# david-cortes/recometrics

Measured on AMD Instinct MI355X. Metric: users/sec evaluated (all metrics, K=10), higher is better.
Workload: dtype f32

## Files before the change

### recometrics_amd/csrc/rm_finalize.hpp

```cpp
#pragma once
#include "rm_device.hpp"
#include <type_traits>

namespace rm {

constexpr int MAX_PARTS = 128;
constexpr int FIN_THREADS = 128;
constexpr int FIN_TOPV = 64;
template <class T> inline size_t finalize_lds_bytes(int K, int n_part) { return (sizeof(T) * (size_t)(K < FIN_TOPV ? K : FIN_TOPV) + 4 * (size_t)n_part) * FIN_THREADS; }

struct AucPart { unsigned long long sum_ranks; double s1, s2; int nvalid, pad; };

template <class T, class S> struct FinalArgs {
    int m, n, K, n_part, req, cumulative, noise, gu, n_slots;
    const int *slot_user, *slot_chunk;
    const int *train_p, *test_p, *test_i; const T *test_v;
    const int *flags, *user_nslots, *uslot_base, *slot_index;
    const int *gj; const long long *grow;
    const Entry<S> *pl; const PartialStat<S> *pst; const unsigned *hist; const S *pos_score;
    const int *pos_item_tab;
    AucPart *auc_part;
    T *heavy_topv;
    unsigned char *heavy_nan;
    const int *heavy_users; int n_heavy;
// ... 10 lines not shown
    int auc_defer_slot0;
    const S *stream_scores; long long stream_ld;
    const S *spos_score; const int *spos_item;
    unsigned *shist;
    int ext_topk; unsigned long long *sel_hi; unsigned *sel_lo; int sel_ld;
    int collected;
    int *noise_flag; Plan *plan;
};

template <class T> __device__ __forceinline__ T qnan();
template <> __device__ __forceinline__ float qnan<float>() { return __int_as_float(0x7fc00000); }
template <> __device__ __forceinline__ double qnan<double>() { return __longlong_as_double(0x7ff8000000000000ll); }

template <class T, class S>
__device__ void fill_user_nan(const FinalArgs<T, S> &a, int u)
{
    T *top8[8] = {a.p, a.tp, a.r, a.ap, a.tap, a.ndcg, a.hit, a.rr};
    for (int q = 0; q < 8; q++) {
        T *arr = top8[q];
        if (!arr) continue;
        if (!a.cumulative) arr[u] = qnan<T>();
        else for (int i = 0; i < a.K; i++) arr[(size_t)u * a.K + i] = qnan<T>();
    }
    if (a.roc) a.roc[u] = qnan<T>();
    if (a.pr) a.pr[u] = qnan<T>();
}

template <class S> __device__ __forceinline__ bool ent_before(const Entry<S> &x, const Entry<S> &y)
{
    return x.s > y.s || (x.s == y.s && x.idx < y.idx);
}

template <class T, class S>
__global__ void k_auc_slots(FinalArgs<T, S> a)
{
    const int slot = blockIdx.x * blockDim.x + threadIdx.x;
    if (slot >= a.stream_slot0) return;
    const int u = a.slot_user[slot], c = a.slot_chunk[slot];
    if (a.flags[u] & UF_ONLY_NDCG) return;
    const int te0 = a.test_p[u], npos = a.test_p[u + 1] - te0;
    const int GUr = a.gu;
    const int g = slot / GUr, ul = slot % GUr;
    const int PLg = (1 << a.gj[g]) - 1;
    const unsigned *H = a.hist + (a.grow[g] + g) * GUr + ul;
    const S *PS = a.pos_score + (a.grow[g] + g) * GUr + ul;
    const int pc = min(POS_CHUNK, npos - c * POS_CHUNK);
    unsigned long long above = 0, sum_ranks = 0;
    double s1 = 0, s2 = 0;
    int nvalid = 0;
    for (int b = PLg; b >= 1; b--) {
        above += H[(size_t)b * GUr];
        const int j = b - 1;
        if (j >= pc) continue;
        const S ps = PS[(size_t)j * GUr];
        if (isinf(ps) && ps > 0) continue;
        const unsigned long long rank = above + 1;
        sum_ranks += rank; nvalid++;
        s1 += 1. / (double)rank;
        s2 += (double)nvalid / (double)rank;
        if (a.rank_sorted) a.rank_sorted[te0 + c * POS_CHUNK + j] = (long long)rank;
    }
    AucPart r; r.sum_ranks = sum_ranks; r.s1 = s1; r.s2 = s2; r.nvalid = nvalid; r.pad = 0;
    a.auc_part[slot] = r;
}

constexpr int MERGE_WAVES = 4;
template <class T, class S>
__global__ __launch_bounds__(MERGE_WAVES * WAVE) void k_merge_positives(FinalArgs<T, S> a, int extra, int slot0)
{
    const int slot = slot0 + __builtin_amdgcn_readfirstlane((int)((blockIdx.x * blockDim.x + threadIdx.x) >> 6)), lane = threadIdx.x & 63;
// ... 673 lines not shown
            if (r > 0 && !(x < pv || (x == pv && t > pi))) return;
            if (!found || x > bv) { found = true; bv = x; bi = t; }
        };
        if (cached) {
            #pragma unroll
            for (int i = 0; i < CACHE; i++) if (lane + WAVE * i < npos) consider(xv[i], lane + WAVE * i);
        } else {
            for (int t = lane; t < npos; t += WAVE) consider(tv[t], t);
        }
        #pragma unroll
        for (int d = 32; d >= 1; d >>= 1) {
            const T ov = __shfl_xor(bv, d); const int oi = __shfl_xor(bi, d); const bool of = __shfl_xor((int)found, d) != 0;
            if (of && (!found || ov > bv || (ov == bv && oi < bi))) { found = true; bv = ov; bi = oi; }
        }
        pv = bv; pi = bi;
        if (lane == 0) out[r] = bv;
    }
    const unsigned long long nm = __ballot(any_nan);
    if (lane == 0) a.heavy_nan[u] = nm ? 1 : 0;
}

template <class T, class S>
__global__ void k_finalize_skipped(FinalArgs<T, S> a)
{
    const int u = blockIdx.x * blockDim.x + threadIdx.x;
    if (u >= a.m || !(a.flags[u] & UF_NAN)) return;
    const int te0 = a.test_p[u], npos = a.test_p[u + 1] - te0;
    if (a.status) a.status[u] = 1;
    Entry<S> *M = a.merged + (size_t)u * a.K;
    for (int i = 0; i < a.K; i++) { M[i].s = (S)qnan<float>(); M[i].idx = -1; }
    fill_user_nan(a, u);
}

template <class T, class S>
__device__ __forceinline__ void finalize_auc(const FinalArgs<T, S> &a, int u, int base, int npos, int C)
{
    const int nsl = a.user_nslots[u];
    unsigned long long sum_ranks = 0; int h = 0; double ap_full = 0;
    for (int c = nsl - 1; c >= 0; c--) {
        const AucPart r = a.auc_part[a.slot_index[base + c]];
        sum_ranks += r.sum_ranks;
        ap_full = nsl == 1 ? r.s2 : ap_full + ((double)h * r.s1 + r.s2);
        h += r.nvalid;
    }
    const unsigned long long P = (unsigned long long)npos, Nneg = (unsigned long long)C - P;
    if (a.roc) a.roc[u] = (T)(1. - (double)(sum_ranks - (P * (P + 1)) / 2) / (double)(P * Nneg));
    if (a.pr) a.pr[u] = (T)(ap_full / (double)npos);
}

template <class T, class S>
__global__ void k_finalize_auc(FinalArgs<T, S> a)
{
    const int slot = a.auc_defer_slot0 + blockIdx.x * blockDim.x + threadIdx.x;
    if (slot >= a.n_slots || a.slot_chunk[slot] != 0) return;
    const int u = a.slot_user[slot];
    const T probe = a.roc ? a.roc[u] : a.pr[u];
    if (probe != probe) return;
    const int npos = a.test_p[u + 1] - a.test_p[u];
    const int C = a.n - (a.train_p[u + 1] - a.train_p[u]);
    finalize_auc(a, u, a.uslot_base[u], npos, C);
}

template <class T, class S>
__global__ void k_finalize(FinalArgs<T, S> a)
{
    extern __shared__ __attribute__((aligned(16))) char fin_smem[];
    T *topv_base = (T *)fin_smem;
    unsigned short *head_base = (unsigned short *)(fin_smem + sizeof(T) * (a.K < FIN_TOPV ? a.K : FIN_TOPV) * FIN_THREADS);
    const int slot = a.fin_slot0 + blockIdx.x * blockDim.x + threadIdx.x;
    if (slot >= a.fin_slot1 || a.slot_chunk[slot] != 0) return;
    const int u = a.slot_user[slot];
    const int K = a.K, n = a.n;
    const int f = a.flags[u];
    const int te0 = a.test_p[u], npos = a.test_p[u + 1] - te0;
    if (a.status) a.status[u] = 1;
    Entry<S> *M = a.merged + (size_t)u * K;
    const bool merged_ready = a.ext_topk || a.collected;
    if (!merged_ready) for (int i = 0; i < K; i++) { M[i].s = (S)qnan<float>(); M[i].idx = -1; }

    const int ntr = a.train_p[u + 1] - a.train_p[u];
    const int C = n - ntr;
    const bool only_ndcg = f & UF_ONLY_NDCG, kleqn = f & UF_KLEQN;
    const int base = a.uslot_base[u];
    const int s0 = a.slot_index[base];
    const int NP = a.n_part;

    unsigned short *head = head_base + threadIdx.x;
    unsigned short *alive = head_base + (size_t)NP * FIN_THREADS + threadIdx.x;
    S vmax = -(S)INFINITY, vmin = (S)INFINITY; bool any_nan = false;
    const Entry<S> *PL = a.pl + (size_t)s0 * NP * K;
    int n_alive = 0;
    for (int q = 0; q < NP; q++) {
        const bool empty = !merged_ready && PL[(size_t)q * K].idx == IDX_EMPTY;
        head[q * FIN_THREADS] = empty ? (unsigned short)K : (unsigned short)0;
        if (!empty) alive[(n_alive++) * FIN_THREADS] = (unsigned short)q;
        const PartialStat<S> ps = a.pst[(size_t)s0 * NP + q];
        vmax = ps.vmax > vmax ? ps.vmax : vmax;
        vmin = ps.vmin < vmin ? ps.vmin : vmin;
        any_nan |= ps.has_nan != 0;
    }
    for (int i = 0; i < (merged_ready ? 0 : K); i++) {
        int best = -1; Entry<S> be; be.s = 0; be.idx = 0;
        for (int t = 0; t < n_alive; t++) {
            const int q = alive[t * FIN_THREADS];
            const int hq = head[q * FIN_THREADS];
            if (hq >= K) continue;
            const Entry<S> e = PL[(size_t)q * K + hq];
            if (best < 0 || ent_before(e, be)) { best = q; be = e; }
        }
        if (best >= 0) head[best * FIN_THREADS]++;
        else be.idx = IDX_EMPTY;
        if (be.idx == IDX_EMPTY) { be.idx = -1; be.s = (S)qnan<float>(); }
        M[i] = be;
    }
    const int W = K < C ? K : C;

    const bool ref_full = ((a.req & RQ_ROC) && !only_ndcg) || K >= C;
    bool invalid = any_nan;
    if (a.noise) invalid |= (vmax == vmin) || isinf(vmax) || isinf(vmin);
    else {
        const S hi = M[0].s, lo = ref_full ? vmin : M[W - 1].s;
        invalid |= isinf(hi) || isinf(lo) || hi == lo || M[W - 1].idx < 0;
    }
    if (invalid) {
        for (int i = 0; i < K; i++) { M[i].s = (S)qnan<float>(); M[i].idx = -1; }
        if (a.rank_sorted) for (int t = 0; t < npos; t++) a.rank_sorted[te0 + t] = 0;
        fill_user_nan(a, u); return;
    }
    if (a.status) a.status[u] = 0;
    if (a.noise_flag) {
        bool zone = false;
        for (int i = 0; i < W; i++) { const S x = M[i].s; zone |= (x < (S)0 ? -x : x) < (S)6.103515625e-05f; }
        if (zone && atomicExch(&a.noise_flag[u], 1) == 0) atomicAdd(&a.plan->n_noise_flagged, 1);
    }

    const int *ti = a.test_i + te0;
    const T *tv = a.test_v ? a.test_v + te0 : nullptr;
    const size_t st = (size_t)u * K;
    T *cp = a.p ? a.p + st : nullptr, *ctp = a.tp ? a.tp + st : nullptr, *cr = a.r ? a.r + st : nullptr;
    T *cap = a.ap ? a.ap + st : nullptr, *ctap = a.tap ? a.tap + st : nullptr, *cndcg = a.ndcg ? a.ndcg + st : nullptr;
    T *chit = a.hit ? a.hit + st : nullptr, *crr = a.rr ? a.rr + st : nullptr;
    const bool cum = a.cumulative;

    const bool top = a.req & (RQ_P | RQ_TP | RQ_R | RQ_AP | RQ_TAP | RQ_NDCG | RQ_HIT | RQ_RR);
    bool walked = false;
    int hits = 0, first = 0x7fffffff;
    double avg_p = 0, dcg = 0;
    if (top && (!kleqn || (a.req & (RQ_AP | RQ_TAP | RQ_RR | RQ_NDCG)))) {
        walked = true;
        for (int ix = 0; ix < W; ix++) {
            const int item = M[ix].idx;
            int lo = 0, hi = npos;
            while (lo < hi) { const int mid = (lo + hi) >> 1; if (ti[mid] < item) lo = mid + 1; else hi = mid; }
            if (lo < npos && ti[lo] == item) {
                hits++;
                avg_p += hits / (double)(ix + 1);
                dcg += tv ? ((double)tv[lo] / a.log2tab[ix]) : 0.;
                first = first < ix ? first : ix;
            }
            if (cum) {
                const int mn = (ix + 1) < npos ? (ix + 1) : npos;
                if (cp) cp[ix] = (T)(hits / (double)(ix + 1));
                if (ctp) ctp[ix] = (T)(hits / (double)mn);
                if (cr) cr[ix] = (T)(hits / (double)npos);
                if (cap) cap[ix] = (T)(avg_p / (double)npos);
                if (ctap) ctap[ix] = (T)(avg_p / (double)mn);
                if (cndcg) cndcg[ix] = (T)dcg;
                if (chit) chit[ix] = (T)(hits > 0);
                if (crr) crr[ix] = (T)(hits ? ((double)1 / (double)(first + 1)) : 0.);
            }
        }
        if (!cum) {
            const int mn = K < npos ? K : npos;
            if (a.p) a.p[u] = (T)((double)hits / (double)K);
            if (a.tp) a.tp[u] = (T)((double)hits / (double)mn);
            if (a.r) a.r[u] = (T)((double)hits / (double)npos);
            if (a.ap) a.ap[u] = (T)(avg_p / (double)npos);
            if (a.tap) a.tap[u] = (T)(avg_p / (double)mn);
            if (a.hit) a.hit[u] = (T)(hits > 0);
            if (a.rr) a.rr[u] = (T)(hits ? (1. / (double)(first + 1)) : 0.);
        } else if (K > C) {
            for (int i = C; i < K; i++) {
                if (cp) cp[i] = qnan<T>(); if (ctp) ctp[i] = qnan<T>(); if (cr) cr[i] = qnan<T>(); if (chit) chit[i] = qnan<T>();
                if (cap) cap[i] = cap[C - 1]; if (ctap) ctap[i] = ctap[C - 1]; if (crr) crr[i] = crr[C - 1]; if (cndcg) cndcg[i] = cndcg[C - 1];
            }
        }
    }

    if (kleqn) {
        if (!cum) {
            if (a.p) a.p[u] = qnan<T>(); if (a.tp) a.tp[u] = qnan<T>(); if (a.r) a.r[u] = qnan<T>(); if (a.hit) a.hit[u] = qnan<T>();
        } else if (!walked) {
            for (int i = 0; i < K; i++) { if (cp) cp[i] = qnan<T>(); if (ctp) ctp[i] = qnan<T>(); if (cr) cr[i] = qnan<T>(); if (chit) chit[i] = qnan<T>(); }
        }
    } else if (only_ndcg) {
        if (!cum) {
            if (a.p) a.p[u] = qnan<T>(); if (a.tp) a.tp[u] = qnan<T>(); if (a.r) a.r[u] = qnan<T>(); if (a.ap) a.ap[u] = qnan<T>();
            if (a.tap) a.tap[u] = qnan<T>(); if (a.hit) a.hit[u] = qnan<T>(); if (a.rr) a.rr[u] = qnan<T>();
        } else {
            for (int i = 0; i < K; i++) {
                if (cp) cp[i] = qnan<T>(); if (ctp) ctp[i] = qnan<T>(); if (cr) cr[i] = qnan<T>(); if (cap) cap[i] = qnan<T>();
                if (ctap) ctap[i] = qnan<T>(); if (chit) chit[i] = qnan<T>(); if (crr) crr[i] = qnan<T>();
            }
        }
    }

    if (only_ndcg) {
        if (a.roc) a.roc[u] = qnan<T>();
        if (a.pr) a.pr[u] = qnan<T>();
    } else if (a.req & (RQ_ROC | RQ_PR)) {
        if (slot >= a.auc_defer_slot0) {
            if (a.roc) a.roc[u] = (T)0;
            if (a.pr) a.pr[u] = (T)0;
        } else finalize_auc(a, u, base, npos, C);
    }

    if (a.ndcg) {
        const int L = K < npos ? K : npos;
        constexpr int TOPV = FIN_TOPV;
        T *topv = topv_base + threadIdx.x;
        bool has_nan_val = false;
        const bool buffered = L <= TOPV;
        auto pick_next = [&](bool have_prev, T pv, int pi, T &ov, int &oi) {
            bool found = false; T bv = 0; int bi = -1;
            for (int t = 0; t < npos; t++) {
                const T x = tv[t];
                if (have_prev && !(x < pv || (x == pv && t > pi))) continue;
                if (!found || x > bv) { found = true; bv = x; bi = t; }
            }
            ov = bv; oi = bi; return found;
        };
        const bool listed = a.heavy_topv && npos > a.heavy_npos && L <= a.heavy_ld;
        const T *hv = listed ? a.heavy_topv + (size_t)u * a.heavy_ld : nullptr;
        if (listed) has_nan_val = a.heavy_nan[u] != 0;
        if (listed && buffered) {
            for (int i = 0; i < L; i++) topv[i * FIN_THREADS] = hv[i];
        } else if (listed) {
        } else if (buffered) {
            int cnt = 0;
            T kth = 0;
            for (int t0 = 0; t0 < npos; t0 += 8) {
                T xb[8];
                #pragma unroll
                for (int q = 0; q < 8; q++) xb[q] = t0 + q < npos ? tv[t0 + q] : (T)0;
                #pragma unroll
                for (int q = 0; q < 8; q++) {
                    if (t0 + q >= npos) break;
                    const T x = xb[q];
                    has_nan_val |= x != x;
                    if (cnt < L || x > kth) {
                        int j = cnt < L ? cnt : L - 1;
                        while (j > 0 && topv[(j - 1) * FIN_THREADS] < x) { topv[j * FIN_THREADS] = topv[(j - 1) * FIN_THREADS]; j--; }
                        topv[j * FIN_THREADS] = x;
                        cnt = cnt < L ? cnt + 1 : cnt;
                        if (cnt == L) kth = topv[(L - 1) * FIN_THREADS];
                    }
                }
            }
        } else {
            for (int t = 0; t < npos; t++) has_nan_val |= tv[t] != tv[t];
        }
        T pv = 0; int pi = -1; bool hp = false;
        auto next_value = [&](int i) -> T {
            if (buffered) return topv[i * FIN_THREADS];
            if (listed) return hv[i];
            T x; int xi; pick_next(hp, pv, pi, x, xi); hp = true; pv = x; pi = xi; return x;
        };
        T vmaxv = 0, vlast = 0;
        if (buffered) { vmaxv = topv[0]; vlast = topv[(L - 1) * FIN_THREADS]; }
        else if (listed) { vmaxv = hv[0]; vlast = hv[L - 1]; }
        else {
            for (int i = 0; i < L; i++) { const T x = next_value(i); if (i == 0) vmaxv = x; vlast = x; }
            hp = false; pv = 0; pi = -1;
        }
        if (has_nan_val || isinf(vmaxv) || isinf(vlast) || vmaxv <= 0) {
            if (!cum) a.ndcg[u] = qnan<T>(); else for (int i = 0; i < K; i++) cndcg[i] = qnan<T>();
            return;
        }
        double idcg = 0;
        if (!cum) {
            for (int ix = 0; ix < L; ix++) {
                const T x = next_value(ix);
                if (!(vlast >= 0) && x <= 0) break;
                idcg += (double)x / a.log2tab[ix];
            }
            a.ndcg[u] = (T)(dcg / idcg);
        } else {
            if (vlast >= 0) {
                for (int ix = 0; ix < L; ix++) {
                    const T x = next_value(ix);
                    idcg += (double)x / a.log2tab[ix];
                    cndcg[ix] = (T)((double)cndcg[ix] / idcg);
                }
            } else {
                int ix = 0;
                for (; ix < L; ix++) {
                    const T x = next_value(ix);
                    if (x < 0) break;
                    idcg += (double)x / a.log2tab[ix];
                    cndcg[ix] = (T)((double)cndcg[ix] / idcg);
                }
                for (; ix < L; ix++) cndcg[ix] = (T)((double)cndcg[ix] / idcg);
            }
            if (npos < K) { const int e = K < C ? K : C; for (int i = npos; i < e; i++) cndcg[i] = cndcg[npos - 1]; }
        }
    }
}

template <class S> struct RecoArgs {
    int m, n, K, n_part;
    const int *flags, *uslot_base, *slot_index, *train_p;
    const Entry<S> *pl; const PartialStat<S> *pst;
    const Entry<S> *merged;
    int *idx; S *score; int *status;
};
constexpr int RECO_THREADS = 128, RECO_CHUNK = 16, RECO_LD = RECO_CHUNK + 1;
template <class S> inline size_t reco_lds_bytes(int n_part, bool merged_ready)
{
    return merged_ready ? 0 : (sizeof(S) + 4) * (size_t)RECO_THREADS * RECO_LD + 4 * (size_t)n_part * RECO_THREADS;
}

template <class S>
__global__ __launch_bounds__(RECO_THREADS) void k_finalize_reco(RecoArgs<S> a)
{
    extern __shared__ __attribute__((aligned(16))) char reco_smem[];
    __shared__ int len_s[RECO_THREADS];
    const int tid = threadIdx.x;
    const long long u0 = (long long)blockIdx.x * RECO_THREADS;
    const int users_here = (int)(a.m - u0 < RECO_THREADS ? a.m - u0 : RECO_THREADS);
    const int u = (int)u0 + tid;
    const int K = a.K, NP = a.n_part;
    const bool active = tid < users_here && (a.flags[u] & UF_ACTIVE);
    int s0 = 0, W = 0, status = 1;
    if (active) {
        s0 = a.slot_index[a.uslot_base[u]];
        const int C = a.n - (a.train_p[u + 1] - a.train_p[u]);
        S vmax = -(S)INFINITY, vmin = (S)INFINITY; bool any_nan = false;
        for (int q = 0; q < NP; q++) {
            const PartialStat<S> ps = a.pst[(size_t)s0 * NP + q];
// ... 66 lines not shown
```

### recometrics_amd/csrc/rm_lib.hip

```cpp
#include <hip/hip_runtime.h>

#include <algorithm>
#include <array>
#include <cmath>
#include <cstdio>
#include <cstring>
#include <cstdlib>
#include <type_traits>
#include <atomic>
#include <chrono>
#include <condition_variable>
#include <csignal>
#include <functional>
#include <limits>
#include <map>
#include <memory>
#include <mutex>
#include <string>
#include <thread>
#include <vector>

#include "../../include/recometrics_hip.h"
#include "rm_device.hpp"
#include "rm_prep.hpp"
#include "rm_launch.hpp"
#include "rm_finalize.hpp"
#include "rm_noise.hpp"

namespace {

using namespace rm;

thread_local std::string g_err;
struct RmError { int code; std::string msg; };

#define HIP_CHECK(expr)                                                                                   \
    do {                                                                                                  \
        hipError_t e_ = (expr);                                                                           \
        if (e_ != hipSuccess)                                                                             \
            throw RmError{e_ == hipErrorOutOfMemory ? RM_ERR_NOMEM : RM_ERR_HIP,                          \
                          std::string(#expr) + ": " + hipGetErrorString(e_)};                             \
    } while (0)

struct Switches {
    bool no_train_bits, no_spec, no_side, ext_topk, no_test_mask, hbm_lists, nsub2, no_pending, no_pos_beside, no_seed, rank_generic,
         no_fused_auc, no_defer_auc, noise_sequential, one_context, noise_per_batch, host_trace, no_pos_flat;
    long long free_mb, stream_budget_mb, noise_budget_mb, lane_cap_min, lane_min_k, lane_cap_set, sample_seed;
    double batch_users;
    std::string splits;
    static bool on(const char *name) { return getenv(name) != nullptr; }
    static long long num(const char *name) { const char *e = getenv(name); return e ? atoll(e) : -1; }
    void load()
    {
        no_train_bits = on("RM_DEBUG_NO_TRAIN_BITS"); no_spec = on("RM_DEBUG_NO_SPEC"); no_side = on("RM_DEBUG_NO_SIDE");
        ext_topk = on("RM_DEBUG_EXT_TOPK"); no_test_mask = on("RM_DEBUG_NO_TEST_MASK");
        hbm_lists = on("RM_DEBUG_HBM_LISTS"); nsub2 = on("RM_DEBUG_NSUB2"); no_pending = on("RM_DEBUG_NO_PENDING");
        no_pos_beside = on("RM_DEBUG_NO_POS_BESIDE"); no_seed = on("RM_DEBUG_NO_SEED");
        rank_generic = on("RM_DEBUG_RANK_GENERIC"); no_fused_auc = on("RM_DEBUG_NO_FUSED_AUC");
        no_defer_auc = on("RM_DEBUG_NO_DEFER_AUC"); noise_sequential = on("RM_DEBUG_NOISE_SEQUENTIAL");
        one_context = on("RM_DEBUG_ONE_CONTEXT"); noise_per_batch = on("RM_DEBUG_NOISE_PER_BATCH"); host_trace = on("RM_HOST_TRACE");
        no_pos_flat = on("RM_DEBUG_NO_POS_FLAT");
        free_mb = num("RM_DEBUG_FREE_MB"); stream_budget_mb = num("RM_STREAM_BUDGET_MB");
        noise_budget_mb = num("RM_NOISE_BUDGET_MB");
        lane_min_k = num("RM_DEBUG_LANE_MIN_K");
        lane_cap_set = num("RM_DEBUG_LANE_CAP");
        sample_seed = num("RM_DEBUG_SAMPLE_SEED");
        lane_cap_min = num("RM_DEBUG_LANE_CAP_MIN");
        const char *b = getenv("RM_BATCH_USERS"); batch_users = b ? atof(b) : 0.0;
        const char *s = getenv("RM_DEBUG_SPLITS"); splits = s ? s : "";
    }
    Switches() { load(); }
};
Switches g_sw;

std::atomic<long long> g_ws_bytes{0};
inline long long debug_free_cap()
{
    return g_sw.free_mb >= 0 ? (g_sw.free_mb << 20) : -1;
}

struct RunTrace {
    std::mutex mu; std::vector<std::pair<const char *, double>> pts; std::chrono::steady_clock::time_point t0 = std::chrono::steady_clock::now();
    void point(const char *what) { std::lock_guard<std::mutex> lk(mu); if (pts.size() > 4096) pts.clear(); pts.emplace_back(what, std::chrono::duration<double, std::milli>(std::chrono::steady_clock::now() - t0).count()); }
};
RunTrace g_run_trace;
#define RM_TRACE_POINT(what) do { if (g_sw.host_trace) g_run_trace.point(what); } while (0)

std::atomic<unsigned long long> g_ws_stamp{1};
struct Workspace {
    struct Buf { void *ptr = nullptr; size_t bytes = 0; unsigned long long stamp = 0; };
    std::map<std::string, Buf> bufs;
    void *get(const std::string &name, size_t bytes)
    {
        bytes = std::max<size_t>(bytes, 256);
// ... 904 lines not shown
            P::set_sync(sl, (int)(g.lds_l - SYNC_BYTES));
            dispatch_sweep(want_auc, false, false, g.nsub, NG, dim3((unsigned)((n_ublocks - u_split - sb.tail_ublocks) * g.n_splits + sb.tail_ublocks * g.tail_splits)), g.lds_total, side.fork(SIDE_SWEEP_FORK), sb);
            side.mark(SIDE_SWEEP_DEEP_DONE);
            dispatch_sweep(want_auc, false, true, g.nsub, NG, dim3((unsigned)((u_split - sl.tail_ublocks) * g.n_splits + sl.tail_ublocks * g.tail_splits)), g.lds_l, stream, sl);
            side.await(SIDE_SWEEP_DEEP_DONE, stream);
            side.enabled = use_side;
        } else {
            dispatch_sweep(want_auc, false, g.list_in_lds, g.nsub, NG, dim3(n_blocks), g.lds_total, stream, sa);
        }
        RM_TRACE_POINT("run: sweep enqueued");
        HIP_CHECK(hipEventRecord(cx.ev[EV_SWEEP_END], stream));
        if (lane_lists) {
            collect = true;
            collect_g = CollectGeom{sa.ublock0, sa.n_ublocks, g.n_splits, g.tail_ublocks, g.tail_splits, g.nsub, GU, P::lanes_per_user, sa.lane_cap, g.part_extra ? g.n_part - 1 : -1};
        }
        tm[4] = g.u_split > 0 ? 2 : 1; tm[5] = g.n_splits; tm[6] = n_blocks; tm[7] = (double)g.lds_total;
        cx.timed_slots = n_slots;
        cx.total_slots = n_slots;
    }

    int stream_parts() const { return (int)cdiv(n, STREAM_RANK_THREADS * STREAM_RANK_ITEMS); }
    void rank_streamed_rows(int r0, int r1, hipStream_t st)
    {
        if (r1 <= r0) return;
        const int parts = stream_parts();
        const int ipt = ((int)cdiv(n, (long long)parts * STREAM_RANK_THREADS) + 7) / 8 * 8;
        hipLaunchKernelGGL((k_rank_streamed<T, T>), dim3((unsigned)((long long)(r1 - r0) * parts)), dim3(STREAM_RANK_THREADS), 0, st, fa, parts, ipt, r0);
    }
    void auc_streamed_rows(int r0, int r1, hipStream_t st)
    {
        if (r1 <= r0) return;
        hipLaunchKernelGGL((k_auc_streamed<T, T>), dim3(cdiv((long long)(r1 - r0) * WAVE, 256)), dim3(256), 0, st, fa, r0, r1);
    }
    void finalize_slots(int s0, int s1, size_t fin_lds)
    {
        if (s1 <= s0) return;
        fa.fin_slot0 = s0; fa.fin_slot1 = s1;
        hipLaunchKernelGGL((k_finalize<T, T>), dim3(cdiv(s1 - s0, FIN_THREADS)), dim3(FIN_THREADS), fin_lds, stream, fa);
    }

    void collect_lists()
    {
        if (!collect) return;
        fa.collected = 1;
        const char *gl = (const char *)glists;
        if (collect_capw(K, collect_g.lane_cap) == 512)
            hipLaunchKernelGGL((k_collect_topk<T, T, ThrT, 512>), dim3(collect_grid(cdiv(n_slots, 4))), dim3(256), 0, stream, fa, collect_g, gl, lane_cnt, (const ThrT *)thr_shared);
        else if (collect_capw(K, collect_g.lane_cap) == 1024)
            hipLaunchKernelGGL((k_collect_topk<T, T, ThrT, 1024>), dim3(collect_grid(cdiv(n_slots, 4))), dim3(256), 0, stream, fa, collect_g, gl, lane_cnt, (const ThrT *)thr_shared);
        else
            hipLaunchKernelGGL((k_collect_topk<T, T, ThrT, 4096>), dim3(collect_grid(n_slots)), dim3(64), 0, stream, fa, collect_g, gl, lane_cnt, (const ThrT *)thr_shared);
    }
    void select_lists()
    {
        if (!(n_slots > 0 && ext_topk)) return;
        int sel_ld = 2;
        while (sel_ld < K) sel_ld <<= 1;
        fa.ext_topk = 1; fa.sel_ld = sel_ld;
        fa.sel_hi = (unsigned long long *)ws.get("sel_hi", sizeof(unsigned long long) * (size_t)n_slots * sel_ld);
        fa.sel_lo = (unsigned *)ws.get("sel_lo", sizeof(unsigned) * (size_t)n_slots * sel_ld);
        hipLaunchKernelGGL((k_select_topk<T, T>), dim3(n_slots), dim3(SELECT_THREADS), 0, stream, fa);
    }

    void finalize_reco()
    {
        fa.n_part = g.n_part; fa.pl = pl; fa.pst = pst;
        fa.stream_slot0 = stream_slot0; fa.stream_scores = stream_scores; fa.stream_ld = stream_ld;
        collect_lists();
        select_lists();
        const bool merged_ready = n_slots > 0 && (collect || ext_topk);
        RecoArgs<T> ra{m, n, K, g.n_part, flags, uslot_base, slot_index, c.train_p, pl, pst, merged_ready ? merged : nullptr,
                       c.topk_idx, c.topk_score, c.status};
        const size_t lds = reco_lds_bytes<T>(g.n_part, merged_ready);
        if (lds > 48 * 1024) HIP_CHECK(hipFuncSetAttribute((const void *)k_finalize_reco<T>, hipFuncAttributeMaxDynamicSharedMemorySize, (int)lds));
        hipLaunchKernelGGL(k_finalize_reco<T>, dim3(cdiv(m, RECO_THREADS)), dim3(RECO_THREADS), lds, stream, ra);
        HIP_CHECK(hipGetLastError());
    }

    void finalize()
    {
        fa.n_part = g.n_part; fa.pl = pl; fa.pst = pst; fa.hist = hist; fa.pos_score = pos_score; fa.pos_item_tab = pos_item;
        fa.stream_slot0 = stream_slot0; fa.stream_scores = stream_scores; fa.stream_ld = stream_ld;
        fa.spos_score = spos_score; fa.spos_item = spos_item; fa.shist = shist;
        fa.rank_generic = (g_sw.rank_generic ? 1 : 0);
        const bool ranks_beside = use_side && n_slots > 0 && want_auc && n_stream > 0;
        bool auc_launch = true;
        if (stream_parts() == 1 && !g_sw.no_fused_auc) {
            fa.fused_auc = 1 | (g.mask_test ? 2 : 0);
            long long top = 1;
            while (top <= hp.max_npos) top <<= 1;
            auc_launch = ext_topk || !(top * (long long)(sizeof(T) / 4) + hp.max_npos + 1 <= STREAM_RANK_LDS / 4);
        }
        hipStream_t rank_stream = stream;
        if (ranks_beside) { rank_stream = side.fork(SIDE_FORK); rank_streamed_rows(0, n_stream, rank_stream); }
        if (g.mask_test) {
            if (n_slots > stream_slot0)
                hipLaunchKernelGGL((k_merge_positives<T, T>), dim3(cdiv(n_slots - stream_slot0, MERGE_WAVES)), dim3(MERGE_WAVES * WAVE), 0, stream, fa, g.n_part - 1, stream_slot0);
            if (ranks_beside && auc_launch) rank_stream = side.fork(SIDE_MERGED);
        }
        if (ranks_beside && auc_launch) auc_streamed_rows(0, n_stream, rank_stream);
        hipLaunchKernelGGL((k_finalize_skipped<T, T>), dim3(cdiv(m, 256)), dim3(256), 0, stream, fa);
        if (side.marked(SIDE_TOP_VALUES)) side.await(SIDE_TOP_VALUES, stream);
        collect_lists();
        select_lists();
        if (n_slots > 0) {
            if (want_auc) {
                if (n_stream > 0 && !ranks_beside) { rank_streamed_rows(0, n_stream, stream); if (auc_launch) auc_streamed_rows(0, n_stream, stream); }
                if (stream_slot0 > 0) hipLaunchKernelGGL((k_auc_slots<T, T>), dim3(cdiv(stream_slot0, 256)), dim3(256), 0, stream, fa);
            }
            const size_t fin_lds = finalize_lds_bytes<T>(K, g.n_part);
            HIP_CHECK(hipFuncSetAttribute((const void *)k_finalize<T, T>, hipFuncAttributeMaxDynamicSharedMemorySize, (int)fin_lds));
            fa.auc_defer_slot0 = n_slots;
            if (ranks_beside && (req & (RQ_ROC | RQ_PR)) && !g_sw.no_defer_auc) {
                fa.auc_defer_slot0 = stream_slot0;
                finalize_slots(0, n_slots, fin_lds);
                side.join(SIDE_JOIN);
                hipLaunchKernelGGL((k_finalize_auc<T, T>), dim3(cdiv(n_slots - stream_slot0, 256)), dim3(256), 0, stream, fa);
            } else if (ranks_beside) {
                finalize_slots(0, stream_slot0, fin_lds);
                side.join(SIDE_JOIN);
                finalize_slots(stream_slot0, n_slots, fin_lds);
            } else finalize_slots(0, n_slots, fin_lds);
        }
        HIP_CHECK(hipGetLastError());
    }

    void export_ranks()
    {
        if (c.topk_idx && !c.reco)
            hipLaunchKernelGGL(k_export_rank<T>, dim3(cdiv((long long)m * K, 256)), dim3(256), 0, stream, m, K, merged, c.topk_idx, c.topk_score, flags);
        if (c.pos_rank)
            hipLaunchKernelGGL(k_export_pos_rank, dim3(cdiv(m, 128)), dim3(128), 0, stream, c.nnz_test, m, c.test_p, flags, pos_order, rank_sorted, c.pos_rank,
                               (want_auc && n_slots > 0) ? 1 : 0, c.status);
        RM_TRACE_POINT("run: finalisation enqueued");
        HIP_CHECK(hipEventRecord(cx.ev[EV_END], stream));
        HIP_CHECK(hipEventRecord(cx.done, stream));
        cx.ev_recorded = true;
        HIP_CHECK(hipGetLastError());
    }
};

// ... 1089 lines not shown
```

Measured before the change: 17.60 million.

## Add LDS-staged finalize kernel fusing AUC slot pass for small-list users

Introduces k_finalize_staged, which cooperatively loads each block's partial top-K lists, stats and test positives into LDS with coalesced batched loads. It then runs the merge, metric and AUC computation from LDS instead of strided per-thread global reads, and computes the AUC partial inline rather than in a separate k_auc_slots pass. The finalize logic is templated over a source abstraction so the generic and staged paths share code, and slot ranges not covered by staged launches fall back to the old kernels. The staged blocks use only 32 threads and large LDS, which may hurt occupancy, and several extra kernel launches are added per range.

```diff
diff --git a/recometrics_amd/csrc/rm_finalize.hpp b/recometrics_amd/csrc/rm_finalize.hpp
--- a/recometrics_amd/csrc/rm_finalize.hpp
+++ b/recometrics_amd/csrc/rm_finalize.hpp
@@ -66,10 +66,10 @@
 }
 
 template <class T, class S>
-__global__ void k_auc_slots(FinalArgs<T, S> a)
-{
-    const int slot = blockIdx.x * blockDim.x + threadIdx.x;
-    if (slot >= a.stream_slot0) return;
+__global__ void k_auc_slots(FinalArgs<T, S> a, int slot0, int slot1)
+{
+    const int slot = slot0 + blockIdx.x * blockDim.x + threadIdx.x;
+    if (slot >= slot1 || slot >= a.stream_slot0) return;
     const int u = a.slot_user[slot], c = a.slot_chunk[slot];
     if (a.flags[u] & UF_ONLY_NDCG) return;
     const int te0 = a.test_p[u], npos = a.test_p[u + 1] - te0;
@@ -809,13 +809,14 @@
     fill_user_nan(a, u);
 }
 
-template <class T, class S>
-__device__ __forceinline__ void finalize_auc(const FinalArgs<T, S> &a, int u, int base, int npos, int C)
-{
-    const int nsl = a.user_nslots[u];
+template <class T, class S, bool OWN = false>
+__device__ __forceinline__ void finalize_auc(const FinalArgs<T, S> &a, int u, int base, int npos, int C, const AucPart &own = AucPart())
+{
+    const int nsl = OWN ? 1 : a.user_nslots[u];
     unsigned long long sum_ranks = 0; int h = 0; double ap_full = 0;
     for (int c = nsl - 1; c >= 0; c--) {
-        const AucPart r = a.auc_part[a.slot_index[base + c]];
+        AucPart r;
+        if (OWN) r = own; else r = a.auc_part[a.slot_index[base + c]];
         sum_ranks += r.sum_ranks;
         ap_full = nsl == 1 ? r.s2 : ap_full + ((double)h * r.s1 + r.s2);
         h += r.nvalid;
@@ -838,40 +839,66 @@
     finalize_auc(a, u, a.uslot_base[u], npos, C);
 }
 
-template <class T, class S>
-__global__ void k_finalize(FinalArgs<T, S> a)
-{
-    extern __shared__ __attribute__((aligned(16))) char fin_smem[];
-    T *topv_base = (T *)fin_smem;
-    unsigned short *head_base = (unsigned short *)(fin_smem + sizeof(T) * (a.K < FIN_TOPV ? a.K : FIN_TOPV) * FIN_THREADS);
-    const int slot = a.fin_slot0 + blockIdx.x * blockDim.x + threadIdx.x;
-    if (slot >= a.fin_slot1 || a.slot_chunk[slot] != 0) return;
-    const int u = a.slot_user[slot];
+template <class T, class S, int LD> struct FinSrcGlobal {
+    static constexpr bool STAGED = false;
+    const Entry<S> *PL; const PartialStat<S> *PST; const int *TI; const T *TV; Entry<S> *M; int K;
+    T *topv_; unsigned short *head_, *alive_;
+    __device__ __forceinline__ Entry<S> pl(int q, int i) const { return PL[(size_t)q * K + i]; }
+    __device__ __forceinline__ int pl_idx(int q, int i) const { return PL[(size_t)q * K + i].idx; }
+    __device__ __forceinline__ PartialStat<S> pst(int q) const { return PST[q]; }
+    __device__ __forceinline__ int ti(int t) const { return TI[t]; }
+    __device__ __forceinline__ T tv(int t) const { return TV[t]; }
+    __device__ __forceinline__ bool has_tv() const { return TV != nullptr; }
+    __device__ __forceinline__ void m_clear() const { for (int i = 0; i < K; i++) { M[i].s = (S)qnan<float>(); M[i].idx = -1; } }
+    __device__ __forceinline__ void m_set(int i, const Entry<S> &e) const { M[i] = e; }
+    __device__ __forceinline__ S m_s(int i) const { return M[i].s; }
+    __device__ __forceinline__ int m_idx(int i) const { return M[i].idx; }
+    __device__ __forceinline__ void m_invalidate() const { m_clear(); }
+    __device__ __forceinline__ void m_commit() const {}
+    __device__ __forceinline__ T &topv(int i) const { return topv_[i * LD]; }
+    __device__ __forceinline__ unsigned short &head(int q) const { return head_[q * LD]; }
+    __device__ __forceinline__ unsigned short &alive(int t) const { return alive_[t * LD]; }
+};
+template <class T, class S, int LD> struct FinSrcStaged {
+    static constexpr bool STAGED = true;
+    const Entry<S> *PL; const PartialStat<S> *PST; const int *TI; const T *TV; Entry<S> *M, *Mg; int K;
+    T *topv_; unsigned short *head_, *alive_;
+    __device__ __forceinline__ Entry<S> pl(int q, int i) const { return PL[q * K + i]; }
+    __device__ __forceinline__ int pl_idx(int q, int i) const { return PL[q * K + i].idx; }
+    __device__ __forceinline__ PartialStat<S> pst(int q) const { return PST[q]; }
+    __device__ __forceinline__ int ti(int t) const { return TI[t]; }
+    __device__ __forceinline__ T tv(int t) const { return TV[t]; }
+    __device__ __forceinline__ bool has_tv() const { return TV != nullptr; }
+    __device__ __forceinline__ void m_clear() const {}
+    __device__ __forceinline__ void m_set(int i, const Entry<S> &e) const { M[i] = e; }
+    __device__ __forceinline__ S m_s(int i) const { return M[i].s; }
+    __device__ __forceinline__ int m_idx(int i) const { return M[i].idx; }
+    __device__ __forceinline__ void m_invalidate() const { for (int i = 0; i < K; i++) { Mg[i].s = (S)qnan<float>(); Mg[i].idx = -1; } }
+    __device__ __forceinline__ void m_commit() const { for (int i = 0; i < K; i++) Mg[i] = M[i]; }
+    __device__ __forceinline__ T &topv(int i) const { return topv_[i * LD]; }
+    __device__ __forceinline__ unsigned short &head(int q) const { return head_[q * LD]; }
+    __device__ __forceinline__ unsigned short &alive(int t) const { return alive_[t * LD]; }
+};
+
+template <class T, class S, class Src>
+__device__ __forceinline__ void finalize_user(const FinalArgs<T, S> &a, const Src &src, int slot, int u, int f, int te0, int npos, int ntr, int base, const AucPart &own)
+{
     const int K = a.K, n = a.n;
-    const int f = a.flags[u];
-    const int te0 = a.test_p[u], npos = a.test_p[u + 1] - te0;
     if (a.status) a.status[u] = 1;
-    Entry<S> *M = a.merged + (size_t)u * K;
-    const bool merged_ready = a.ext_topk || a.collected;
-    if (!merged_ready) for (int i = 0; i < K; i++) { M[i].s = (S)qnan<float>(); M[i].idx = -1; }
-
-    const int ntr = a.train_p[u + 1] - a.train_p[u];
+    const bool merged_ready = !Src::STAGED && (a.ext_topk || a.collected);
+    if (!merged_ready) src.m_clear();
+
     const int C = n - ntr;
     const bool only_ndcg = f & UF_ONLY_NDCG, kleqn = f & UF_KLEQN;
-    const int base = a.uslot_base[u];
-    const int s0 = a.slot_index[base];
     const int NP = a.n_part;
 
-    unsigned short *head = head_base + threadIdx.x;
-    unsigned short *alive = head_base + (size_t)NP * FIN_THREADS + threadIdx.x;
     S vmax = -(S)INFINITY, vmin = (S)INFINITY; bool any_nan = false;
-    const Entry<S> *PL = a.pl + (size_t)s0 * NP * K;
     int n_alive = 0;
     for (int q = 0; q < NP; q++) {
-        const bool empty = !merged_ready && PL[(size_t)q * K].idx == IDX_EMPTY;
-        head[q * FIN_THREADS] = empty ? (unsigned short)K : (unsigned short)0;
-        if (!empty) alive[(n_alive++) * FIN_THREADS] = (unsigned short)q;
-        const PartialStat<S> ps = a.pst[(size_t)s0 * NP + q];
+        const bool empty = !merged_ready && src.pl_idx(q, 0) == IDX_EMPTY;
+        src.head(q) = empty ? (unsigned short)K : (unsigned short)0;
+        if (!empty) src.alive(n_alive++) = (unsigned short)q;
+        const PartialStat<S> ps = src.pst(q);
         vmax = ps.vmax > vmax ? ps.vmax : vmax;
         vmin = ps.vmin < vmin ? ps.vmin : vmin;
         any_nan |= ps.has_nan != 0;
@@ -879,16 +906,16 @@
     for (int i = 0; i < (merged_ready ? 0 : K); i++) {
         int best = -1; Entry<S> be; be.s = 0; be.idx = 0;
         for (int t = 0; t < n_alive; t++) {
-            const int q = alive[t * FIN_THREADS];
-            const int hq = head[q * FIN_THREADS];
+            const int q = src.alive(t);
+            const int hq = src.head(q);
             if (hq >= K) continue;
-            const Entry<S> e = PL[(size_t)q * K + hq];
+            const Entry<S> e = src.pl(q, hq);
             if (best < 0 || ent_before(e, be)) { best = q; be = e; }
         }
-        if (best >= 0) head[best * FIN_THREADS]++;
+        if (best >= 0) src.head(best)++;
         else be.idx = IDX_EMPTY;
         if (be.idx == IDX_EMPTY) { be.idx = -1; be.s = (S)qnan<float>(); }
-        M[i] = be;
+        src.m_set(i, be);
     }
     const int W = K < C ? K : C;
 
@@ -896,23 +923,23 @@
     bool invalid = any_nan;
     if (a.noise) invalid |= (vmax == vmin) || isinf(vmax) || isinf(vmin);
     else {
-        const S hi = M[0].s, lo = ref_full ? vmin : M[W - 1].s;
-        invalid |= isinf(hi) || isinf(lo) || hi == lo || M[W - 1].idx < 0;
+        const S hi = src.m_s(0), lo = ref_full ? vmin : src.m_s(W - 1);
+        invalid |= isinf(hi) || isinf(lo) || hi == lo || src.m_idx(W - 1) < 0;
     }
     if (invalid) {
-        for (int i = 0; i < K; i++) { M[i].s = (S)qnan<float>(); M[i].idx = -1; }
+        src.m_invalidate();
         if (a.rank_sorted) for (int t = 0; t < npos; t++) a.rank_sorted[te0 + t] = 0;
         fill_user_nan(a, u); return;
     }
+    src.m_commit();
     if (a.status) a.status[u] = 0;
     if (a.noise_flag) {
         bool zone = false;
-        for (int i = 0; i < W; i++) { const S x = M[i].s; zone |= (x < (S)0 ? -x : x) < (S)6.103515625e-05f; }
+        for (int i = 0; i < W; i++) { const S x = src.m_s(i); zone |= (x < (S)0 ? -x : x) < (S)6.103515625e-05f; }
         if (zone && atomicExch(&a.noise_flag[u], 1) == 0) atomicAdd(&a.plan->n_noise_flagged, 1);
     }
 
-    const int *ti = a.test_i + te0;
-    const T *tv = a.test_v ? a.test_v + te0 : nullptr;
+    const bool has_tv = src.has_tv();
     const size_t st = (size_t)u * K;
     T *cp = a.p ? a.p + st : nullptr, *ctp = a.tp ? a.tp + st : nullptr, *cr = a.r ? a.r + st : nullptr;
     T *cap = a.ap ? a.ap + st : nullptr, *ctap = a.tap ? a.tap + st : nullptr, *cndcg = a.ndcg ? a.ndcg + st : nullptr;
@@ -926,13 +953,13 @@
     if (top && (!kleqn || (a.req & (RQ_AP | RQ_TAP | RQ_RR | RQ_NDCG)))) {
         walked = true;
         for (int ix = 0; ix < W; ix++) {
-            const int item = M[ix].idx;
+            const int item = src.m_idx(ix);
             int lo = 0, hi = npos;
-            while (lo < hi) { const int mid = (lo + hi) >> 1; if (ti[mid] < item) lo = mid + 1; else hi = mid; }
-            if (lo < npos && ti[lo] == item) {
+            while (lo < hi) { const int mid = (lo + hi) >> 1; if (src.ti(mid) < item) lo = mid + 1; else hi = mid; }
+            if (lo < npos && src.ti(lo) == item) {
                 hits++;
                 avg_p += hits / (double)(ix + 1);
-                dcg += tv ? ((double)tv[lo] / a.log2tab[ix]) : 0.;
+                dcg += has_tv ? ((double)src.tv(lo) / a.log2tab[ix]) : 0.;
                 first = first < ix ? first : ix;
             }
             if (cum) {
@@ -989,19 +1016,18 @@
         if (slot >= a.auc_defer_slot0) {
             if (a.roc) a.roc[u] = (T)0;
             if (a.pr) a.pr[u] = (T)0;
-        } else finalize_auc(a, u, base, npos, C);
+        } else finalize_auc<T, S, Src::STAGED>(a, u, base, npos, C, own);
     }
 
     if (a.ndcg) {
         const int L = K < npos ? K : npos;
         constexpr int TOPV = FIN_TOPV;
-        T *topv = topv_base + threadIdx.x;
         bool has_nan_val = false;
         const bool buffered = L <= TOPV;
         auto pick_next = [&](bool have_prev, T pv, int pi, T &ov, int &oi) {
             bool found = false; T bv = 0; int bi = -1;
             for (int t = 0; t < npos; t++) {
-                const T x = tv[t];
+                const T x = src.tv(t);
                 if (have_prev && !(x < pv || (x == pv && t > pi))) continue;
                 if (!found || x > bv) { found = true; bv = x; bi = t; }
             }
@@ -1011,7 +1037,7 @@
         const T *hv = listed ? a.heavy_topv + (size_t)u * a.heavy_ld : nullptr;
         if (listed) has_nan_val = a.heavy_nan[u] != 0;
         if (listed && buffered) {
-            for (int i = 0; i < L; i++) topv[i * FIN_THREADS] = hv[i];
+            for (int i = 0; i < L; i++) src.topv(i) = hv[i];
         } else if (listed) {
         } else if (buffered) {
             int cnt = 0;
@@ -1019,7 +1045,7 @@
             for (int t0 = 0; t0 < npos; t0 += 8) {
                 T xb[8];
                 #pragma unroll
-                for (int q = 0; q < 8; q++) xb[q] = t0 + q < npos ? tv[t0 + q] : (T)0;
+                for (int q = 0; q < 8; q++) xb[q] = t0 + q < npos ? src.tv(t0 + q) : (T)0;
                 #pragma unroll
                 for (int q = 0; q < 8; q++) {
                     if (t0 + q >= npos) break;
@@ -1027,24 +1053,24 @@
                     has_nan_val |= x != x;
                     if (cnt < L || x > kth) {
                         int j = cnt < L ? cnt : L - 1;
-                        while (j > 0 && topv[(j - 1) * FIN_THREADS] < x) { topv[j * FIN_THREADS] = topv[(j - 1) * FIN_THREADS]; j--; }
-                        topv[j * FIN_THREADS] = x;
+                        while (j > 0 && src.topv(j - 1) < x) { src.topv(j) = src.topv(j - 1); j--; }
+                        src.topv(j) = x;
                         cnt = cnt < L ? cnt + 1 : cnt;
-                        if (cnt == L) kth = topv[(L - 1) * FIN_THREADS];
+                        if (cnt == L) kth = src.topv(L - 1);
                     }
                 }
             }
         } else {
-            for (int t = 0; t < npos; t++) has_nan_val |= tv[t] != tv[t];
+            for (int t = 0; t < npos; t++) has_nan_val |= src.tv(t) != src.tv(t);
         }
         T pv = 0; int pi = -1; bool hp = false;
         auto next_value = [&](int i) -> T {
-            if (buffered) return topv[i * FIN_THREADS];
+            if (buffered) return src.topv(i);
             if (listed) return hv[i];
             T x; int xi; pick_next(hp, pv, pi, x, xi); hp = true; pv = x; pi = xi; return x;
         };
         T vmaxv = 0, vlast = 0;
-        if (buffered) { vmaxv = topv[0]; vlast = topv[(L - 1) * FIN_THREADS]; }
+        if (buffered) { vmaxv = src.topv(0); vlast = src.topv(L - 1); }
         else if (listed) { vmaxv = hv[0]; vlast = hv[L - 1]; }
         else {
             for (int i = 0; i < L; i++) { const T x = next_value(i); if (i == 0) vmaxv = x; vlast = x; }
@@ -1082,6 +1108,165 @@
             if (npos < K) { const int e = K < C ? K : C; for (int i = npos; i < e; i++) cndcg[i] = cndcg[npos - 1]; }
         }
     }
+}
+
+template <class T, class S>
+__global__ void k_finalize(FinalArgs<T, S> a)
+{
+    extern __shared__ __attribute__((aligned(16))) char fin_smem[];
+    T *topv_base = (T *)fin_smem;
+    unsigned short *head_base = (unsigned short *)(fin_smem + sizeof(T) * (a.K < FIN_TOPV ? a.K : FIN_TOPV) * FIN_THREADS);
+    const int slot = a.fin_slot0 + blockIdx.x * blockDim.x + threadIdx.x;
+    if (slot >= a.fin_slot1 || a.slot_chunk[slot] != 0) return;
+    const int u = a.slot_user[slot];
+    const int f = a.flags[u];
+    const int te0 = a.test_p[u], npos = a.test_p[u + 1] - te0;
+    const int ntr = a.train_p[u + 1] - a.train_p[u];
+    const int base = a.uslot_base[u];
+    const int s0 = a.slot_index[base];
+    const int NP = a.n_part;
+    FinSrcGlobal<T, S, FIN_THREADS> src;
+    src.PL = a.pl + (size_t)s0 * NP * a.K; src.PST = a.pst + (size_t)s0 * NP;
+    src.TI = a.test_i + te0; src.TV = a.test_v ? a.test_v + te0 : nullptr;
+    src.M = a.merged + (size_t)u * a.K; src.K = a.K;
+    src.topv_ = topv_base + threadIdx.x;
+    src.head_ = head_base + threadIdx.x;
+    src.alive_ = head_base + (size_t)NP * FIN_THREADS + threadIdx.x;
+    finalize_user(a, src, slot, u, f, te0, npos, ntr, base, AucPart());
+}
+
+constexpr int STG_THREADS = 32;
+constexpr int STG_BATCH = 16;
+constexpr size_t STG_LDS_BUDGET = 64 * 1024;
+struct StagedLayout { unsigned pl, pst, m, tv, topv, ti, meta, head, total; };
+template <class T, class S>
+__host__ __device__ inline StagedLayout staged_layout(int K, int n_part, int cap, bool has_tv)
+{
+    auto up = [](size_t x) { return (x + 15) / 16 * 16; };
+    StagedLayout L; size_t at = 0;
+    L.pl = (unsigned)at;   at = up(at + sizeof(Entry<S>) * (size_t)STG_THREADS * n_part * K);
+    L.m = (unsigned)at;    at = up(at + sizeof(Entry<S>) * (size_t)STG_THREADS * K);
+    L.pst = (unsigned)at;  at = up(at + sizeof(PartialStat<S>) * (size_t)STG_THREADS * n_part);
+    L.tv = (unsigned)at;   at = up(at + (has_tv ? sizeof(T) * (size_t)STG_THREADS * (cap + 1) : 0));
+    L.topv = (unsigned)at; at = up(at + sizeof(T) * (size_t)(K < FIN_TOPV ? K : FIN_TOPV) * STG_THREADS);
+    L.ti = (unsigned)at;   at = up(at + 4 * (size_t)STG_THREADS * (cap + 1));
+    L.meta = (unsigned)at; at = up(at + 4 * (size_t)2 * STG_THREADS);
+    L.head = (unsigned)at; at = up(at + 2 * (size_t)2 * n_part * STG_THREADS);
+    L.total = (unsigned)at;
+    return L;
+}
+template <class T, class S> inline size_t staged_lds_bytes(int K, int n_part, int cap, bool has_tv)
+{
+    const size_t lists = sizeof(Entry<S>) * (size_t)STG_THREADS * (size_t)n_part * (size_t)K;
+    if (lists > STG_LDS_BUDGET) return lists;
+    return staged_layout<T, S>(K, n_part, cap, has_tv).total;
+}
+
+template <class T, class S>
+__global__ __launch_bounds__(STG_THREADS) void k_finalize_staged(FinalArgs<T, S> a, int lgcap, int do_auc)
+{
+    extern __shared__ __attribute__((aligned(16))) char stg_smem[];
+    const int K = a.K, NP = a.n_part, tid = threadIdx.x;
+    const int cap = 1 << lgcap, row_ld = cap + 1;
+    const bool has_tv = a.test_v != nullptr;
+    const StagedLayout L = staged_layout<T, S>(K, NP, cap, has_tv);
+    Entry<S> *sPL = (Entry<S> *)(stg_smem + L.pl), *sM = (Entry<S> *)(stg_smem + L.m);
+    PartialStat<S> *sPST = (PartialStat<S> *)(stg_smem + L.pst);
+    T *sTV = (T *)(stg_smem + L.tv), *sTopv = (T *)(stg_smem + L.topv);
+    int *sTI = (int *)(stg_smem + L.ti), *sTe0 = (int *)(stg_smem + L.meta), *sNpos = sTe0 + STG_THREADS;
+    unsigned short *sHead = (unsigned short *)(stg_smem + L.head);
+
+    const int slot_b = a.fin_slot0 + blockIdx.x * STG_THREADS;
+    const int here = min(STG_THREADS, a.fin_slot1 - slot_b);
+    const int slot = slot_b + tid;
+    const bool mine = tid < here;
+
+    const int u = a.slot_user[mine ? slot : slot_b];
+    auto copy_flat = [&](const void *gsrc, void *ldst, int words) __attribute__((always_inline)) {
+        const unsigned long long *src = (const unsigned long long *)gsrc;
+        unsigned long long *dst = (unsigned long long *)ldst;
+        for (int i0 = 0; i0 < words; i0 += STG_BATCH * STG_THREADS) {
+            unsigned long long r[STG_BATCH];
+            #pragma unroll
+            for (int q = 0; q < STG_BATCH; q++) { const int i = i0 + q * STG_THREADS + tid; r[q] = src[i < words ? i : words - 1]; }
+            #pragma unroll
+            for (int q = 0; q < STG_BATCH; q++) { const int i = i0 + q * STG_THREADS + tid; if (i < words) dst[i] = r[q]; }
+        }
+    };
+    copy_flat(a.pl + (size_t)slot_b * NP * K, sPL, here * NP * K * (int)(sizeof(Entry<S>) / 8));
+    copy_flat(a.pst + (size_t)slot_b * NP, sPST, here * NP * (int)(sizeof(PartialStat<S>) / 8));
+    const int f = a.flags[u];
+    const int te0 = a.test_p[u], te1 = a.test_p[u + 1];
+    const int ntr = a.train_p[u + 1] - a.train_p[u];
+    const int npos = te1 - te0;
+    sTe0[tid] = mine ? te0 : 0;
+    sNpos[tid] = mine ? (npos < cap ? npos : cap) : 0;
+    __syncthreads();
+    for (int i0 = 0; i0 < STG_THREADS * cap; i0 += STG_BATCH * STG_THREADS) {
+        int ri[STG_BATCH]; T rv[STG_BATCH];
+        #pragma unroll
+        for (int q = 0; q < STG_BATCH; q++) {
+            const int i = i0 + q * STG_THREADS + tid;
+            const int sl = (i >> lgcap) & (STG_THREADS - 1), t = i & (cap - 1);
+            const int e = sTe0[sl] + (t < sNpos[sl] ? t : 0);
+            ri[q] = a.test_i[e];
+            rv[q] = has_tv ? a.test_v[e] : (T)0;
+        }
+        #pragma unroll
+        for (int q = 0; q < STG_BATCH; q++) {
+            const int i = i0 + q * STG_THREADS + tid;
+            const int sl = i >> lgcap, t = i & (cap - 1);
+            if (sl < STG_THREADS && t < sNpos[sl]) { sTI[sl * row_ld + t] = ri[q]; if (has_tv) sTV[sl * row_ld + t] = rv[q]; }
+        }
+    }
+    __syncthreads();
+    if (!mine) return;
+
+    AucPart part = AucPart();
+    if (do_auc && !(f & UF_ONLY_NDCG)) {
+        const int GUr = a.gu;
+        const int g = slot / GUr, ul = slot % GUr;
+        const int PLg = (1 << a.gj[g]) - 1;
+        const unsigned *H = a.hist + (a.grow[g] + g) * GUr + ul;
+        const S *PS = a.pos_score + (a.grow[g] + g) * GUr + ul;
+        const int pc = min(POS_CHUNK, npos);
+        unsigned long long above = 0, sum_ranks = 0;
+        double s1 = 0, s2 = 0;
+        int nvalid = 0;
+        for (int b0 = PLg; b0 >= 1; b0 -= STG_BATCH) {
+            unsigned hb[STG_BATCH]; S pb[STG_BATCH];
+            #pragma unroll
+            for (int q = 0; q < STG_BATCH; q++) {
+                const int b = b0 - q >= 1 ? b0 - q : 1;
+                hb[q] = H[(size_t)b * GUr]; pb[q] = PS[(size_t)(b - 1) * GUr];
+            }
+            #pragma unroll
+            for (int q = 0; q < STG_BATCH; q++) {
+                const int b = b0 - q;
+                if (b < 1) break;
+                above += hb[q];
+                const int j = b - 1;
+                if (j >= pc) continue;
+                const S ps = pb[q];
+                if (isinf(ps) && ps > 0) continue;
+                const unsigned long long rank = above + 1;
+                sum_ranks += rank; nvalid++;
+                s1 += 1. / (double)rank;
+                s2 += (double)nvalid / (double)rank;
+                if (a.rank_sorted) a.rank_sorted[te0 + j] = (long long)rank;
+            }
+        }
+        part.sum_ranks = sum_ranks; part.s1 = s1; part.s2 = s2; part.nvalid = nvalid; part.pad = 0;
+        a.auc_part[slot] = part;
+    }
+
+    FinSrcStaged<T, S, STG_THREADS> src;
+    src.PL = sPL + (size_t)tid * NP * K; src.PST = sPST + (size_t)tid * NP;
+    src.TI = sTI + tid * row_ld; src.TV = has_tv ? sTV + tid * row_ld : nullptr;
+    src.M = sM + (size_t)tid * K; src.Mg = a.merged + (size_t)u * K; src.K = K;
+    src.topv_ = sTopv + tid;
+    src.head_ = sHead + tid; src.alive_ = sHead + (size_t)NP * STG_THREADS + tid;
+    finalize_user(a, src, slot, u, f, te0, npos, ntr, 0, part);
 }
 
 template <class S> struct RecoArgs {
diff --git a/recometrics_amd/csrc/rm_lib.hip b/recometrics_amd/csrc/rm_lib.hip
--- a/recometrics_amd/csrc/rm_lib.hip
+++ b/recometrics_amd/csrc/rm_lib.hip
@@ -44,7 +44,7 @@
 
 struct Switches {
     bool no_train_bits, no_spec, no_side, ext_topk, no_test_mask, hbm_lists, nsub2, no_pending, no_pos_beside, no_seed, rank_generic,
-         no_fused_auc, no_defer_auc, noise_sequential, one_context, noise_per_batch, host_trace, no_pos_flat;
+         no_fused_auc, no_defer_auc, noise_sequential, one_context, noise_per_batch, host_trace, no_pos_flat, fin_generic;
     long long free_mb, stream_budget_mb, noise_budget_mb, lane_cap_min, lane_min_k, lane_cap_set, sample_seed;
     double batch_users;
     std::string splits;
@@ -60,6 +60,7 @@
         no_defer_auc = on("RM_DEBUG_NO_DEFER_AUC"); noise_sequential = on("RM_DEBUG_NOISE_SEQUENTIAL");
         one_context = on("RM_DEBUG_ONE_CONTEXT"); noise_per_batch = on("RM_DEBUG_NOISE_PER_BATCH"); host_trace = on("RM_HOST_TRACE");
         no_pos_flat = on("RM_DEBUG_NO_POS_FLAT");
+        fin_generic = on("RM_DEBUG_FIN_GENERIC");
         free_mb = num("RM_DEBUG_FREE_MB"); stream_budget_mb = num("RM_STREAM_BUDGET_MB");
         noise_budget_mb = num("RM_NOISE_BUDGET_MB");
         lane_min_k = num("RM_DEBUG_LANE_MIN_K");
@@ -1030,11 +1031,46 @@
         if (r1 <= r0) return;
         hipLaunchKernelGGL((k_auc_streamed<T, T>), dim3(cdiv((long long)(r1 - r0) * WAVE, 256)), dim3(256), 0, st, fa, r0, r1);
     }
+    struct StagedRange { int s0, s1, lgcap; };
+    std::vector<StagedRange> staged;
+    void plan_staged()
+    {
+        staged.clear();
+        if (g_sw.fin_generic || n_slots == 0 || collect || ext_topk || K > FIN_TOPV || hp.n_slots != hp.n_active) return;
+        const bool has_tv = c.test_v != nullptr;
+        auto add = [&](int j0, int j1, int lgcap) {
+            const int s0 = std::min(hp.class_offset[j0], stream_slot0), s1 = std::min(hp.class_offset[j1], stream_slot0);
+            if (s1 <= s0 || staged_lds_bytes<T, T>(K, g.n_part, 1 << lgcap, has_tv) > STG_LDS_BUDGET) return;
+            staged.push_back(StagedRange{s0, s1, lgcap});
+        };
+        if (hp.max_npos <= POS_CHUNK) add(0, 1, 6);
+        add(1, 5, 4); add(5, 6, 5); add(6, MAX_J + 1, 6);
+    }
+    void launch_staged()
+    {
+        for (const StagedRange &r : staged) {
+            const size_t lds = staged_lds_bytes<T, T>(K, g.n_part, 1 << r.lgcap, c.test_v != nullptr);
+            HIP_CHECK(hipFuncSetAttribute((const void *)k_finalize_staged<T, T>, hipFuncAttributeMaxDynamicSharedMemorySize, (int)lds));
+            fa.fin_slot0 = r.s0; fa.fin_slot1 = r.s1;
+            hipLaunchKernelGGL((k_finalize_staged<T, T>), dim3(cdiv(r.s1 - r.s0, STG_THREADS)), dim3(STG_THREADS), lds, stream, fa, r.lgcap, want_auc ? 1 : 0);
+        }
+    }
+    template <class F> void generic_pieces(int s0, int s1, F launch)
+    {
+        int at = s0;
+        for (const StagedRange &r : staged) {
+            if (r.s1 <= at || r.s0 >= s1) continue;
+            if (r.s0 > at) launch(at, r.s0);
+            at = std::max(at, r.s1);
+        }
+        if (at < s1) launch(at, s1);
+    }
     void finalize_slots(int s0, int s1, size_t fin_lds)
     {
-        if (s1 <= s0) return;
-        fa.fin_slot0 = s0; fa.fin_slot1 = s1;
-        hipLaunchKernelGGL((k_finalize<T, T>), dim3(cdiv(s1 - s0, FIN_THREADS)), dim3(FIN_THREADS), fin_lds, stream, fa);
+        generic_pieces(s0, s1, [&](int lo, int hi) {
+            fa.fin_slot0 = lo; fa.fin_slot1 = hi;
+            hipLaunchKernelGGL((k_finalize<T, T>), dim3(cdiv(hi - lo, FIN_THREADS)), dim3(FIN_THREADS), fin_lds, stream, fa);
+        });
     }
 
     void collect_lists()
@@ -1091,12 +1127,16 @@
         }
         hipStream_t rank_stream = stream;
         if (ranks_beside) { rank_stream = side.fork(SIDE_FORK); rank_streamed_rows(0, n_stream, rank_stream); }
+        plan_staged();
+        const bool merged_fork = g.mask_test && ranks_beside && auc_launch;
+        if (!merged_fork) launch_staged();
         if (g.mask_test) {
             if (n_slots > stream_slot0)
                 hipLaunchKernelGGL((k_merge_positives<T, T>), dim3(cdiv(n_slots - stream_slot0, MERGE_WAVES)), dim3(MERGE_WAVES * WAVE), 0, stream, fa, g.n_part - 1, stream_slot0);
             if (ranks_beside && auc_launch) rank_stream = side.fork(SIDE_MERGED);
         }
         if (ranks_beside && auc_launch) auc_streamed_rows(0, n_stream, rank_stream);
+        if (merged_fork) launch_staged();
         hipLaunchKernelGGL((k_finalize_skipped<T, T>), dim3(cdiv(m, 256)), dim3(256), 0, stream, fa);
         if (side.marked(SIDE_TOP_VALUES)) side.await(SIDE_TOP_VALUES, stream);
         collect_lists();
@@ -1104,7 +1144,7 @@
         if (n_slots > 0) {
             if (want_auc) {
                 if (n_stream > 0 && !ranks_beside) { rank_streamed_rows(0, n_stream, stream); if (auc_launch) auc_streamed_rows(0, n_stream, stream); }
-                if (stream_slot0 > 0) hipLaunchKernelGGL((k_auc_slots<T, T>), dim3(cdiv(stream_slot0, 256)), dim3(256), 0, stream, fa);
+                generic_pieces(0, stream_slot0, [&](int lo, int hi) { hipLaunchKernelGGL((k_auc_slots<T, T>), dim3(cdiv(hi - lo, 256)), dim3(256), 0, stream, fa, lo, hi); });
             }
             const size_t fin_lds = finalize_lds_bytes<T>(K, g.n_part);
             HIP_CHECK(hipFuncSetAttribute((const void *)k_finalize<T, T>, hipFuncAttributeMaxDynamicSharedMemorySize, (int)fin_lds));
```

Result: slower. 16.93 million (-3.8%).
